# ScissorJack-ever/AlayaLite

Measured on AMD Instinct MI355X. Metric: QPS @ recall@10>=0.95, GIST-960 L2, 1M base / 1k queries, higher is better.
Workload: dtype f32

## Files before the change

### alayalite_amd/csrc/capi.cpp

```cpp
#include "../../include/alaya_hip.h"

#include <hip/hip_runtime_api.h>

#include <algorithm>
#include <cfloat>
#include <cmath>
#include <cstring>
#include <memory>
#include <mutex>
#include <stdexcept>
#include <limits>
#include <string>
#include <thread>
#include <vector>

#include "build_kernels.h"
#include "graph_update.h"
#include "hnsw_build.h"
#include "flat_bound.h"
#include "flat_kernels.h"
#include <cstdlib>
#include "screen_bound.h"
#include "search_kernels.h"

// ... 85 lines not shown
  int sq8_order = 2;
  uint32_t code_stride = 0;
  DevBuf codes, sq_min, sq_max, rr_q_buf, sq_ids, sq_d;
  DevBuf norms, cand_d, cand_i, flat_tau, flag_buf, iota, flat_q;
  DevBuf flat_bias;
  int flat_contraction = -1;
  bool norms_ready = false;
  DevBuf flat_tiles, tiles_cand, tiles_qexp;
  bool tiles_ready = false;
  int tiles_exp = 0;
  int tiles_metric = -1;
  float max_norm = 0.f;
  DevBuf work, overflow, dirty, stab, q_buf, id_buf, dist_buf, cnt_buf, dlist_buf, dout_buf;
  size_t overflow_clean = 0;
  size_t stab_clean = 0;
  uint32_t hash_log2_override = 0;
  int helpers_mode = -1;
  DevBuf help_stats;
  uint64_t help_stats_slots = 0;
  struct ScreenCopy {
    DevBuf rows, err;
    uint64_t cap = 0;
    bool ready = false;
    bool failed = false;
  };
  ScreenCopy screen_copy[2];
  uint32_t screen_format = 0;
  DevBuf screen_stats;
  uint64_t screen_stats_slots = 0;
  uint32_t last_grid = 0, last_waves = 0;
  uint32_t last_lds = 0, last_hash_log2 = 0, last_compact = 0, last_per_cu = 0, last_scout = 0;
  DevBuf scout_stats;
  uint64_t scout_stats_slots = 0;
  int visited_mode_override = 0;
  int num_cus = 0;
  uint64_t capacity = 0;
  std::unique_ptr<alaya_amd::HostGraph> upd_graph;
  std::unique_ptr<alaya_amd::RowMirror> upd_rows;
  std::unique_ptr<alaya_amd::UpdateContext> upd_ctx;
  hipStream_t stream = nullptr;
  hipEvent_t scratch_ev = nullptr;
  hipStream_t scratch_stream = nullptr;
  bool scratch_used = false;
  uint64_t device_bytes() const {
    return base.bytes + valid.bytes + l0.bytes + levels.bytes + upper_off.bytes +
           upper_edges.bytes + eps.bytes + overflow.bytes + dirty.bytes + stab.bytes + codes.bytes + sq_min.bytes +
           sq_max.bytes;
  }
};

namespace {

void set_device(const alaya_index *ix) { hip_check(hipSetDevice(ix->device), "hipSetDevice"); }

void scratch_acquire(alaya_index *ix, hipStream_t s) {
  if (ix->scratch_used && ix->scratch_stream != s)
    hip_check(hipStreamWaitEvent(s, ix->scratch_ev, 0), "hipStreamWaitEvent");
}
void scratch_release(alaya_index *ix, hipStream_t s) {
  hip_check(hipEventRecord(ix->scratch_ev, s), "hipEventRecord");
  ix->scratch_stream = s;
  ix->scratch_used = true;
}
void scratch_suspect(alaya_index *ix) {
  ix->overflow_clean = 0;
  ix->stab_clean = 0;
// ... 209 lines not shown
    } else if (force != 0) {
      int b1 = 0;
      const size_t probe = search_wave_lds_bytes(ix->stride, ef, 12, true);
      hip_check(search_occupancy(resolve_search_variant(r), p.ip, 1, probe, &b1), "occupancy");
      const uint64_t resident1 = static_cast<uint64_t>(std::max(1, b1)) * static_cast<uint64_t>(stream_cus(ix, stream));
      if (nq > resident1 && 2 * nq <= 3 * resident1) r.want |= kModeTwoWaves;
    }
  }
  if (ensure_screen(ix, p, p.sq8_order == 0 && plain, stream)) r.want |= kModeScreen;
  return r;
}

struct SearchPlan {
  const alaya_amd::SearchVariant *variant;
  int W;
  size_t lds;
  int grid;
  int per_cu;
};

uint32_t scout_default(uint32_t dim) { return (dim == 768 || dim == 960) ? alaya_amd::kScoutOn : 0u; }

uint32_t scout_requested(uint32_t dim) {
  const char *e = std::getenv("ALAYA_SEARCH_SCOUT");
  const int asked = e && e[0] ? std::atoi(e) : -1;
  uint32_t f = asked < 0 ? scout_default(dim) : (asked == 1 ? alaya_amd::kScoutOn : (asked == 2 ? alaya_amd::kScoutOn | alaya_amd::kScoutVerify : 0u));
  if (f != 0u) {
    const char *m = std::getenv("ALAYA_SEARCH_SCOUT_MISS");
    if (m && std::atoi(m) != 0) f |= alaya_amd::kScoutMiss;
  }
  return f;
}

SearchPlan plan_search(alaya_index *ix, SearchParams &p, alaya_amd::SearchRequest r, uint64_t nq, uint32_t ef,
                       hipStream_t stream) {
  using namespace alaya_amd;
  SearchPlan plan{};
  for (;;) {
    plan.variant = &resolve_search_variant(r);
    const int mode = plan.variant->mode;
    if ((r.want & kModeStamp) != 0 && (mode & kModeStamp) == 0)
      throw ArgError("no stamped search kernel for dim " + std::to_string(ix->dim) +
                     (p.sq8_order ? " SQ8 (order " + std::to_string(p.sq8_order) + ")" : std::string(" f32")) +
                     ": see the variant list in search_variants.h");
    p.help = (mode & kModeHelp) != 0;
    p.two_waves = (mode & kModeTwoWaves) != 0;
    p.screen = (mode & kModeScreen) != 0 ? ix->screen_format : 0u;
    plan.W = p.help ? 4 : search_waves(p);
    while (!p.help && plan.W > 1 && static_cast<uint64_t>(plan.W) > nq) plan.W /= 2;
    p.hash_log2 = size_visited(ix, p, *plan.variant, nq, ef, plan.W);
    const bool compact = p.vis_rbits != kVisWide;
    p.wave_lds = static_cast<uint32_t>(search_wave_lds_bytes(ix->stride, ef, p.hash_log2, compact, p.sq8_order));
    bool fits = true;
    if (p.help) {
      const size_t need = static_cast<size_t>(plan.W) * kHelpMemoSlots * ix->R * 8;
      const size_t q_bytes = search_query_lds_bytes(ix->stride, p.sq8_order);
      if (q_bytes >= need) {
        p.memo_off = 0;
      } else if (p.wave_lds >= q_bytes + 3 * 64 * 4 + need) {
        p.memo_off = static_cast<uint32_t>(q_bytes + 3 * 64 * 4);
      } else {
        fits = false;
      }
    }
    plan.lds = search_shared_lds_bytes(ix->stride, p.sq8_order != 0) + static_cast<size_t>(plan.W) * p.wave_lds +
               (p.help ? kHelpBoardBytes : 0);
    if (!p.help || (fits && plan.lds <= kLdsPerCu)) break;
    r.want &= ~kModeHelp;
  }
  if (plan.lds > kLdsPerCu) throw ArgError("ef / dim too large for the LDS budget");
  int per_cu = 0;
  hip_check(search_occupancy(*plan.variant, p.ip, plan.W, plan.lds, &per_cu), "occupancy");
  per_cu = static_cast<int>(std::max<uint64_t>(1, std::min<uint64_t>(per_cu, max_search_waves_per_cu() / plan.W)));
  const uint64_t cus = static_cast<uint64_t>(stream_cus(ix, stream));
  const uint64_t blocks_needed = p.help ? static_cast<uint64_t>(per_cu) * cus : (nq + plan.W - 1) / plan.W;
  plan.grid = static_cast<int>(std::max<uint64_t>(1, std::min<uint64_t>(blocks_needed, static_cast<uint64_t>(per_cu) * cus)));
  plan.per_cu = per_cu;
  p.scout = 0u;
  const uint32_t scout = scout_requested(ix->dim);
  if (scout != 0u && p.screen == 3u && !p.ip && !p.two_waves && !p.help && plan.W == 1 && ix->R <= kScoutR &&
      (plan.variant->mode & ~kModeScreen) == 0 && search_has_two_waves(ix->dim, p.sq8_order, ix->generic) &&
      !helpers_requested(ix, p, nq, cus)) {
    SearchRequest r2 = r;
    r2.want |= kModeTwoWaves;
    const SearchVariant &v2 = resolve_search_variant(r2);
    const size_t lds2 = plan.lds + kScoutBoardBytes;
    int per_cu2 = 0;
    if (v2.mode == (kModeScreen | kModeTwoWaves) && lds2 <= kLdsPerCu)
      hip_check(search_occupancy(v2, false, 2, lds2, &per_cu2), "occupancy");
    if (per_cu2 >= per_cu && nq <= static_cast<uint64_t>(per_cu) * cus) {
      plan.variant = &v2;
      plan.lds = lds2;
      p.scout = scout;
      if (const char *e = std::getenv("ALAYA_SEARCH_SCOUT_GRID"))
        plan.grid = std::max(1, std::min(plan.grid, std::atoi(e)));
    }
  }
  return plan;
}

void do_search(alaya_index *ix, const float *d_q, uint64_t nq, uint32_t k, uint32_t ef,
               uint32_t *d_ids, float *d_dists, uint32_t *d_cnt, hipStream_t stream,
               uint64_t *d_stamps = nullptr, bool sq8 = false, uint32_t fill_id = 0) {
  if (!ix->base.ptr) throw ArgError("index has no base vectors");
  if (!ix->has_graph) throw ArgError("index has no graph");
  if (ef == 0) throw ArgError("ef must be >= 1");
  if (k == 0 || nq == 0) return;
  if (ix->graph_n > ix->n) throw ArgError("graph has more nodes than base vectors");
  SearchParams p = base_params(ix);
  p.l0 = ix->l0.as<uint32_t>();
  p.R = ix->R;
  p.dedup_edges = ix->dedup;
  p.levels = ix->has_overlay ? ix->levels.as<uint32_t>() : nullptr;
  p.upper_off = ix->upper_off.as<uint64_t>();
  p.upper_edges = ix->upper_edges.as<uint32_t>();
  p.upper_R = ix->upper_R;
  p.ep = ix->ep;
  p.eps = ix->eps.as<uint32_t>();
  p.n_eps = ix->n_eps;
  p.queries = d_q;
  p.nq = nq;
  p.q_stride = ix->dim;
  p.k = k;
  p.ef = ef;
  p.out_ids = d_ids;
  p.out_dists = d_dists;
// ... 2 lines not shown
  p.fill_id = fill_id;
  if (sq8) {
    if (!ix->has_sq8) throw ArgError("index has no SQ8 codes");
    p.sq8_order = ix->sq8_order;
    p.codes = ix->codes.as<uint8_t>();
    p.code_stride = ix->code_stride;
    p.sq_min = ix->sq_min.as<float>();
    p.sq_max = ix->sq_max.as<float>();
  }
  p.stab_log2 = spill_table_log2(p.sq8_order, std::max<uint32_t>(1, ceil_log2(std::max<uint64_t>(ix->n, 2))), ef);
  if (const char *e = std::getenv("ALAYA_HELP_FLAGS")) p.help_flags = static_cast<uint32_t>(std::strtoul(e, nullptr, 10));
  const SearchPlan plan = plan_search(ix, p, search_request(ix, p, nq, ef, stream), nq, ef, stream);
  if (p.screen >= 2) {
    p.screen_u8 = ix->screen_copy[1].rows.as<uint8_t>();
  } else if (p.screen) {
    p.screen_rows = ix->screen_copy[0].rows.as<uint16_t>();
    p.screen_err = ix->screen_copy[0].err.as<float>();
  }
  scratch_acquire(ix, stream);
  const uint64_t searchers = static_cast<uint64_t>(plan.grid) * plan.W;
  prepare_spill(ix, p, searchers, stream);
  ix->last_grid = static_cast<uint32_t>(plan.grid);
  const int wg_waves = p.scout ? 2 * plan.W : plan.W;
  ix->last_waves = static_cast<uint32_t>(wg_waves);
  ix->last_lds = static_cast<uint32_t>(plan.lds);
  ix->last_hash_log2 = p.hash_log2;
  ix->last_compact = p.vis_rbits != alaya_amd::kVisWide ? 1u : 0u;
  ix->last_per_cu = static_cast<uint32_t>(plan.per_cu);
  ix->last_scout = p.scout;
  ix->scout_stats_slots = p.scout ? searchers : 0;
  if (p.scout) {
    ix->scout_stats.reserve(searchers * 16);
    p.scout_stats = ix->scout_stats.as<uint32_t>();
  }
  ix->help_stats_slots = p.help ? searchers : 0;
  if (p.help) {
    ix->help_stats.reserve(searchers * 12);
    p.help_stats = ix->help_stats.as<uint32_t>();
  }
  ix->screen_stats_slots = p.screen ? searchers : 0;
  if (p.screen) {
    ix->screen_stats.reserve(searchers * 8);
    p.screen_stats = ix->screen_stats.as<uint32_t>();
  }
  ix->work.reserve(4);
  p.work_counter = ix->work.as<uint32_t>();
  hip_check(hipMemsetAsync(p.work_counter, 0, 4, stream), "hipMemsetAsync");
  hip_check(alaya_amd::launch_search(*plan.variant, p, plan.grid, wg_waves, plan.lds, stream), "search launch");
  scratch_release(ix, stream);
}

uint32_t screen_default(uint32_t dim) {
  return (dim == 512 || dim == 768 || dim == 960 || dim == 1024) ? 3u : 0u;
}

void screen_fill(alaya_index *ix, uint32_t format, uint64_t first, uint64_t count, hipStream_t stream) {
  alaya_index::ScreenCopy &c = ix->screen_copy[format - 1];
  hip_check(format == 2 ? alaya_amd::launch_screen_rows_u8(ix->base.as<float>(), first, count, ix->stride,
                                                           c.rows.as<uint8_t>(), stream)
                        : alaya_amd::launch_screen_rows(ix->base.as<float>(), first, count, ix->stride,
                                                        c.rows.as<uint16_t>(), c.err.as<float>(), stream),
            "screening copy");
}

bool ensure_screen(alaya_index *ix, const SearchParams &p, bool eligible, hipStream_t stream) {
  ix->screen_format = 0;
  if (!eligible || !alaya_amd::search_has_screen(ix->dim, p.sq8_order, ix->generic, p.ip)) return false;
// ... 1458 lines not shown
}

int alaya_index_last_plan(const alaya_index *ix, uint32_t *lds_bytes, uint32_t *hash_log2, uint32_t *compact,
                          uint32_t *groups_per_cu, uint32_t *scout) {
  return guarded([&] {
    if (!ix) throw ArgError("null index");
    if (lds_bytes) *lds_bytes = ix->last_lds;
    if (hash_log2) *hash_log2 = ix->last_hash_log2;
    if (compact) *compact = ix->last_compact;
    if (groups_per_cu) *groups_per_cu = ix->last_per_cu;
    if (scout) *scout = ix->last_scout;
  });
}

int alaya_index_scout_stats(alaya_index *ix, uint64_t *expansions, uint64_t *hits, uint64_t *records,
                            uint64_t *mismatches) {
  return guarded_scratch(ix, [&] {
    if (!ix) throw ArgError("null index");
    uint64_t t[4] = {0, 0, 0, 0};
    if (ix->scout_stats_slots) {
      set_device(ix);
      scratch_drain(ix);
      std::vector<uint32_t> h(4 * ix->scout_stats_slots);
      hip_check(hipMemcpy(h.data(), ix->scout_stats.ptr, h.size() * 4, hipMemcpyDeviceToHost), "D2H");
      for (uint64_t i = 0; i < h.size(); ++i) t[i & 3] += h[i];
    }
    if (expansions) *expansions = t[0];
    if (hits) *hits = t[1];
    if (records) *records = t[2];
    if (mismatches) *mismatches = t[3];
  });
}

int alaya_index_set_helpers(alaya_index *ix, int mode) {
  return guarded([&] {
    if (!ix) throw ArgError("null index");
    if (mode < -1 || mode > 1) throw ArgError("helpers mode must be -1 (automatic), 0 (off) or 1 (on)");
    ix->helpers_mode = mode;
  });
}

int alaya_index_help_stats(alaya_index *ix, uint64_t *memo_dists, uint64_t *memo_expansions, uint64_t *helper_rows) {
  return guarded_scratch(ix, [&] {
    if (!ix) throw ArgError("null index");
    uint64_t m = 0, x = 0, r = 0;
    if (ix->help_stats_slots) {
      set_device(ix);
      scratch_drain(ix);
      std::vector<uint32_t> h(3 * ix->help_stats_slots);
      hip_check(hipMemcpy(h.data(), ix->help_stats.ptr, h.size() * 4, hipMemcpyDeviceToHost), "D2H");
      for (uint64_t i = 0; i < ix->help_stats_slots; ++i) {
        m += h[3 * i];
        x += h[3 * i + 1];
        r += h[3 * i + 2];
      }
    }
    if (memo_dists) *memo_dists = m;
    if (memo_expansions) *memo_expansions = x;
    if (helper_rows) *helper_rows = r;
  });
}

int alaya_screen_lower_bound(const float *d_tilde, const float *e_row, uint64_t n, uint32_t dim, float *out) {
  return guarded([&] {
    if (n && (!d_tilde || !e_row || !out)) throw ArgError("invalid arguments");
    for (uint64_t i = 0; i < n; ++i) out[i] = alaya_amd::screen_lower_bound(d_tilde[i], e_row[i], dim);
// ... 156 lines not shown
```

### alayalite_amd/csrc/pybind_module.cpp

```cpp
#include <pybind11/numpy.h>
#include <pybind11/pybind11.h>
#include <pybind11/stl.h>

#include <algorithm>
#include <cmath>
#include <cstring>
#include <fstream>
#include <memory>
#include <queue>
#include <stdexcept>
#include <string>
#include <vector>

#include "../../include/alaya_hip.h"

extern "C" int alaya_index_flat_diag(alaya_index *, const float *, uint64_t, uint32_t, int, uint32_t *, float *,
                                     uint32_t *, uint32_t *, void *);
#include "host_distance.h"

namespace py = pybind11;

namespace alaya_py {

enum class IndexType { FLAT = 0, HNSW = 1, NSG = 2, FUSION = 3, QG = 4 };
// ... 241 lines not shown
    upload();
  }

  uint32_t get_data_dim() const { return dim_; }

  py::array last_counters() const {
    py::array_t<uint32_t> out({static_cast<py::ssize_t>(last_counters_.size() / 4), static_cast<py::ssize_t>(4)});
    std::memcpy(out.mutable_data(), last_counters_.data(), last_counters_.size() * 4);
    return out;
  }
  void set_hash_log2(uint32_t v) { check(alaya_index_set_hash_log2(ix_, v)); }
  void set_visited_mode(int m) { check(alaya_index_set_visited_mode(ix_, m)); }
  void set_helpers(int m) { check(alaya_index_set_helpers(ix_, m)); }
  py::tuple last_launch() {
    uint32_t g = 0, w = 0;
    check(alaya_index_last_launch(ix_, &g, &w));
    return py::make_tuple(g, w);
  }
  py::tuple help_stats() {
    uint64_t m = 0, x = 0, r = 0;
    check(alaya_index_help_stats(ix_, &m, &x, &r));
    return py::make_tuple(m, x, r);
  }
  py::tuple screen_stats() {
    uint64_t a = 0, b = 0;
    check(alaya_index_screen_stats(ix_, &a, &b));
    return py::make_tuple(a, b);
  }
  py::tuple scout_stats() {
    uint64_t e = 0, h = 0, r = 0, m = 0;
    check(alaya_index_scout_stats(ix_, &e, &h, &r, &m));
    return py::make_tuple(e, h, r, m);
  }
  py::dict last_plan() {
    uint32_t g = 0, w = 0, lds = 0, hl = 0, c = 0, pc = 0, sc = 0;
    check(alaya_index_last_launch(ix_, &g, &w));
    check(alaya_index_last_plan(ix_, &lds, &hl, &c, &pc, &sc));
    py::dict d;
    d["workgroups"] = g;
    d["waves_per_group"] = w;
    d["lds_bytes"] = lds;
    d["hash_log2"] = hl;
    d["compact"] = c != 0;
    d["groups_per_cu"] = pc;
    d["scout"] = sc;
    return d;
  }
  void set_rerank_mode(int m) {
    if (m != 1 && m != 2) throw std::invalid_argument("rerank mode must be 1 (reference) or 2 (corrected)");
    rerank_mode_ = m;
  }
  int rerank_mode() const { return rerank_mode_; }
  py::array device_distances(py::array queries, py::array_t<uint32_t> ids) {
    py::array q = prepare_queries(queries);
    py::array_t<uint32_t, py::array::c_style | py::array::forcecast> idc(ids);
    const uint64_t nq = q.shape(0);
    const uint32_t n = static_cast<uint32_t>(idc.size());
    py::array_t<float> out({static_cast<py::ssize_t>(nq), static_cast<py::ssize_t>(n)});
    check(alaya_index_distances(ix_, static_cast<const float *>(q.data()), nq, idc.data(), n,
                                out.mutable_data()));
    return out;
  }
  py::tuple graph_arrays() {
    if (!graph_) throw std::runtime_error("index is not fitted");
    sync_graph();
    uint64_t n, nue;
    uint32_t R, upper_R, ep, max_level, n_eps;
    int has_overlay;
    check(alaya_graph_info(graph_, &n, &R, &has_overlay, &upper_R, &ep, &max_level, &nue, &n_eps));
    py::array_t<uint32_t> l0({static_cast<py::ssize_t>(n), static_cast<py::ssize_t>(R)});
    py::array_t<uint32_t> levels(static_cast<py::ssize_t>(has_overlay ? n : 0));
    py::array_t<uint64_t> off(static_cast<py::ssize_t>(has_overlay ? n : 0));
    py::array_t<uint32_t> ue(static_cast<py::ssize_t>(nue));
    py::array_t<uint32_t> eps(static_cast<py::ssize_t>(n_eps));
    check(alaya_graph_export(graph_, l0.mutable_data(), levels.mutable_data(), off.mutable_data(),
                             ue.mutable_data(), eps.mutable_data()));
    return py::make_tuple(l0, has_overlay ? py::object(levels) : py::none(),
                          has_overlay ? py::object(off) : py::none(), ue, ep, upper_R, eps);
// ... 514 lines not shown
    check(alaya_index_flat_last_contraction(ix_, &c));
    return c;
  }
  void flat_diag(uintptr_t q, uint64_t nq, uint32_t k, int ablate, uintptr_t ids, uintptr_t dists,
                 uintptr_t flags, uintptr_t mc, uintptr_t stream) {
    check(alaya_index_flat_diag(ix_, reinterpret_cast<const float *>(q), nq, k, ablate,
                                reinterpret_cast<uint32_t *>(ids), reinterpret_cast<float *>(dists),
                                reinterpret_cast<uint32_t *>(flags), reinterpret_cast<uint32_t *>(mc),
                                reinterpret_cast<void *>(stream)));
  }
  void set_hash_log2(uint32_t v) { check(alaya_index_set_hash_log2(ix_, v)); }
  void set_visited_mode(int m) { check(alaya_index_set_visited_mode(ix_, m)); }
  void set_helpers(int m) { check(alaya_index_set_helpers(ix_, m)); }
  py::tuple last_launch() {
    uint32_t g = 0, w = 0;
    check(alaya_index_last_launch(ix_, &g, &w));
    return py::make_tuple(g, w);
  }
  py::tuple help_stats() {
    uint64_t m = 0, x = 0, r = 0;
    check(alaya_index_help_stats(ix_, &m, &x, &r));
    return py::make_tuple(m, x, r);
  }
  py::tuple screen_stats() {
    uint64_t a = 0, b = 0;
    check(alaya_index_screen_stats(ix_, &a, &b));
    return py::make_tuple(a, b);
  }
  py::tuple scout_stats() {
    uint64_t e = 0, h = 0, r = 0, m = 0;
    check(alaya_index_scout_stats(ix_, &e, &h, &r, &m));
    return py::make_tuple(e, h, r, m);
  }
  py::dict last_plan() {
    uint32_t g = 0, w = 0, lds = 0, hl = 0, c = 0, pc = 0, sc = 0;
    check(alaya_index_last_launch(ix_, &g, &w));
    check(alaya_index_last_plan(ix_, &lds, &hl, &c, &pc, &sc));
    py::dict d;
    d["workgroups"] = g;
    d["waves_per_group"] = w;
    d["lds_bytes"] = lds;
    d["hash_log2"] = hl;
    d["compact"] = c != 0;
    d["groups_per_cu"] = pc;
    d["scout"] = sc;
    return d;
  }
  py::tuple profile_search(py::array_t<float, py::array::c_style | py::array::forcecast> q, uint32_t k,
                           uint32_t ef, int space) {
    const uint64_t nq = q.shape(0);
    py::array_t<uint32_t> ids({static_cast<py::ssize_t>(nq), static_cast<py::ssize_t>(k)});
    py::array_t<uint32_t> c({static_cast<py::ssize_t>(nq), static_cast<py::ssize_t>(4)});
    py::array_t<uint64_t> st({static_cast<py::ssize_t>(nq), static_cast<py::ssize_t>(8)});
    check(alaya_index_profile_search(ix_, q.data(), nq, k, ef, space, ids.mutable_data(), c.mutable_data(),
                                     st.mutable_data()));
    return py::make_tuple(ids, c, st);
  }
  uint64_t device_bytes() const {
    uint64_t b = 0;
    check(alaya_index_info(ix_, nullptr, nullptr, nullptr, nullptr, &b));
    return b;
  }

 private:
  alaya_index *ix_ = nullptr;
};

}

PYBIND11_MODULE(_alayalitepy, m) {
  using namespace alaya_py;
  m.doc() = "AlayaLite MI355X engine";
  m.attr("__version__") = "0.1.0-mi355x";

  py::enum_<IndexType>(m, "IndexType")
      .value("FLAT", IndexType::FLAT)
      .value("HNSW", IndexType::HNSW)
      .value("NSG", IndexType::NSG)
// ... 32 lines not shown
      .def_readwrite("data_type_", &IndexParams::data_type_)
      .def_readwrite("id_type_", &IndexParams::id_type_)
      .def_readwrite("quantization_type_", &IndexParams::quantization_type_)
      .def_readwrite("metric_", &IndexParams::metric_)
      .def_readwrite("capacity_", &IndexParams::capacity_);

  py::class_<PyIndexInterface, std::shared_ptr<PyIndexInterface>>(m, "PyIndexInterface")
      .def(py::init<IndexParams>(), py::arg("params"))
      .def("to_string", &PyIndexInterface::to_string)
      .def("fit", &PyIndexInterface::fit, py::arg("vectors"), py::arg("ef_construction"), py::arg("num_threads"),
           py::arg("builder") = "host")
      .def("search", &PyIndexInterface::search, py::arg("query"), py::arg("topk"), py::arg("ef"))
      .def("get_data_by_id", &PyIndexInterface::get_data_by_id, py::arg("id"))
      .def("insert", &PyIndexInterface::insert, py::arg("insert_data"), py::arg("ef"))
      .def("remove", &PyIndexInterface::remove, py::arg("id"))
      .def("batch_search", &PyIndexInterface::batch_search, py::arg("queries"), py::arg("topk"),
           py::arg("ef"), py::arg("num_threads"))
      .def("batch_search_with_distance", &PyIndexInterface::batch_search_with_distance,
           py::arg("queries"), py::arg("topk"), py::arg("ef"), py::arg("num_threads"))
      .def("exact_search", &PyIndexInterface::exact_search, py::arg("queries"), py::arg("topk"))
      .def("save", &PyIndexInterface::save, py::arg("index_path"), py::arg("data_path"),
           py::arg("quant_path") = std::string())
      .def("load", &PyIndexInterface::load, py::arg("index_path"), py::arg("data_path"),
           py::arg("quant_path") = std::string())
      .def("get_data_dim", &PyIndexInterface::get_data_dim)
      .def("last_counters", &PyIndexInterface::last_counters)
      .def("set_hash_log2", &PyIndexInterface::set_hash_log2)
      .def("set_visited_mode", &PyIndexInterface::set_visited_mode)
      .def("set_helpers", &PyIndexInterface::set_helpers)
      .def("last_launch", &PyIndexInterface::last_launch)
      .def("help_stats", &PyIndexInterface::help_stats)
      .def("screen_stats", &PyIndexInterface::screen_stats)
      .def("scout_stats", &PyIndexInterface::scout_stats)
      .def("last_plan", &PyIndexInterface::last_plan)
      .def("set_rerank_mode", &PyIndexInterface::set_rerank_mode)
      .def("rerank_mode", &PyIndexInterface::rerank_mode)
      .def("device_distances", &PyIndexInterface::device_distances)
      .def("graph_arrays", &PyIndexInterface::graph_arrays);


  py::class_<Graph, std::shared_ptr<Graph>>(m, "Graph")
      .def_static("build", &Graph::build, py::arg("data"), py::arg("metric") = 0, py::arg("R") = 32u,
                  py::arg("ef_construction") = 100u, py::arg("num_threads") = 1u, py::arg("seed") = 100u)
      .def_static("load", &Graph::load, py::arg("path"), py::arg("id_bytes") = 4)
      .def_static("from_arrays", &Graph::from_arrays, py::arg("l0"), py::arg("levels"), py::arg("upper_off"),
                  py::arg("upper_edges"), py::arg("upper_R"), py::arg("ep"), py::arg("eps") = py::none())
      .def("save", &Graph::save, py::arg("path"), py::arg("id_bytes") = 4, py::arg("capacity") = 0u)
      .def("arrays", &Graph::arrays);
  py::class_<DeviceIndex, std::shared_ptr<DeviceIndex>>(m, "DeviceIndex")
      .def(py::init<int>(), py::arg("device") = 0)
      .def("set_base", &DeviceIndex::set_base, py::arg("rows"), py::arg("metric") = 0, py::arg("valid") = py::none())
      .def("set_graph", &DeviceIndex::set_graph)
      .def("build_graph", &DeviceIndex::build_graph, py::arg("R") = 32, py::arg("ef_construction") = 100,
           py::arg("seed") = 100, py::arg("batch_div") = 0, py::arg("max_batch") = 0, py::arg("refine") = 2)
      .def("search", &DeviceIndex::search, py::arg("queries"), py::arg("k"), py::arg("ef"))
      .def("search_device", &DeviceIndex::search_device)
      .def("shard_search_device", &DeviceIndex::shard_search_device)
      .def("distances", &DeviceIndex::distances)
      .def("set_hash_log2", &DeviceIndex::set_hash_log2)
      .def("set_visited_mode", &DeviceIndex::set_visited_mode)
      .def("set_helpers", &DeviceIndex::set_helpers)
      .def("last_launch", &DeviceIndex::last_launch)
      .def("help_stats", &DeviceIndex::help_stats)
      .def("screen_stats", &DeviceIndex::screen_stats)
      .def("scout_stats", &DeviceIndex::scout_stats)
      .def("last_plan", &DeviceIndex::last_plan)
      .def("flat_search", &DeviceIndex::flat_search, py::arg("queries"), py::arg("k"))
      .def("flat_search_device", &DeviceIndex::flat_search_device)
      .def("flat_diag", &DeviceIndex::flat_diag)
      .def("flat_contraction", &DeviceIndex::flat_contraction)
      .def("search_sq8_device", &DeviceIndex::search_sq8_device)
      .def("shard_search_sq8_device", &DeviceIndex::shard_search_sq8_device)
      .def("set_sq8", &DeviceIndex::set_sq8, py::arg("codes"), py::arg("min"), py::arg("max"), py::arg("order") = 2)
      .def("search_sq8", &DeviceIndex::search_sq8, py::arg("queries"), py::arg("k"), py::arg("ef"),
           py::arg("rerank") = 1, py::arg("rerank_queries") = py::none())
      .def("profile_search", &DeviceIndex::profile_search, py::arg("q"), py::arg("k"), py::arg("ef"),
           py::arg("space") = 0)
      .def("device_bytes", &DeviceIndex::device_bytes);
  m.def("sq8_train", [](py::array_t<float, py::array::c_style | py::array::forcecast> data) {
    const uint32_t d = static_cast<uint32_t>(data.shape(1));
    py::array_t<float> mn(d), mx(d);
    check(alaya_sq8_train(data.data(), data.shape(0), d, mn.mutable_data(), mx.mutable_data()));
    return py::make_tuple(mn, mx);
  });
  m.def("sq8_encode", [](py::array_t<float, py::array::c_style | py::array::forcecast> data,
                         py::array_t<float, py::array::c_style | py::array::forcecast> mn,
                         py::array_t<float, py::array::c_style | py::array::forcecast> mx, uint32_t threads) {
    py::array_t<uint8_t> codes({data.shape(0), data.shape(1)});
    check(alaya_sq8_encode(data.data(), data.shape(0), static_cast<uint32_t>(data.shape(1)), mn.data(), mx.data(),
                           codes.mutable_data(), threads));
    return codes;
  }, py::arg("data"), py::arg("min"), py::arg("max"), py::arg("num_threads") = 1u);
  m.def("host_sq8_order", &host_sq8_order);
  m.def("build_info", [] { return std::string(alaya_build_info()); });
  m.def("screen_lower_bound", [](py::array_t<float, py::array::c_style | py::array::forcecast> d_tilde,
                                 py::array_t<float, py::array::c_style | py::array::forcecast> e_row, uint32_t dim) {
    if (d_tilde.size() != e_row.size()) throw std::invalid_argument("d_tilde and e_row differ in size");
    py::array_t<float> out(d_tilde.size());
// ... 86 lines not shown
```

### alayalite_amd/csrc/search_kernels.h

```cpp
#pragma once
#include <hip/hip_runtime_api.h>

#include <cstddef>
#include <cstdint>

#include "search_variants.h"

namespace alaya_amd {

struct SearchParams {
  const float *base;
  uint64_t n;
  uint32_t dim;
  uint32_t stride;
  const uint32_t *valid;
  bool ip;
  bool generic;
  const uint32_t *l0;
  uint32_t R;
  bool dedup_edges;
  const uint32_t *levels;
  const uint64_t *upper_off;
  const uint32_t *upper_edges;
  uint32_t upper_R;
// ... 11 lines not shown
  uint32_t fill_id;
  uint32_t *work_counter;
  uint32_t *overflow_bits;
  uint32_t *dirty_words;
  uint32_t dirty_cap;
  uint32_t wave_lds;
  uint32_t hash_log2;
  uint32_t vis_rbits;
  uint32_t vis_lbits;
  uint32_t vis_max_disp;
  uint32_t vis_limit;
  uint16_t *spill_table;
  uint32_t stab_log2;
  uint32_t stab_rbits;
  uint32_t spill_flags;
  uint64_t *stamps;
  int sq8_order;
  const uint8_t *codes;
  uint32_t code_stride;
  const float *sq_min;
  const float *sq_max;
  uint32_t help;
  uint32_t help_flags;
  uint32_t memo_off;
  uint32_t two_waves;
  uint32_t *help_stats;
  uint32_t screen;
  const uint16_t *screen_rows;
  const float *screen_err;
  const uint8_t *screen_u8;
  uint32_t *screen_stats;
  uint32_t scout;
  uint32_t *scout_stats;
};
constexpr uint32_t kScoutOn = 1, kScoutVerify = 2, kScoutMiss = 4;
constexpr uint32_t kScoutSlots = 3;
constexpr uint32_t kScoutR = 32;
constexpr size_t kScoutBoardBytes = kScoutSlots * (kScoutR * 4 + 8 + 4) + 20;

struct RerankParams {
  const uint32_t *search_ids;
  uint32_t k;
  uint32_t n_src;
  uint32_t n_take;
  uint32_t zeros;
  uint32_t fill_id;
  uint32_t *out_ids;
  float *out_dists;
};

constexpr uint32_t kVisWide = 0xffffffffu;
constexpr size_t kHelpBoardBytes = 256;
#ifndef ALAYA_HELP_DEPTH
#define ALAYA_HELP_DEPTH 1
#endif
constexpr size_t kHelpMemoSlots = ALAYA_HELP_DEPTH + 1;
constexpr uint32_t kStabBucket = 8;
inline size_t visited_table_bytes(uint32_t hash_log2, bool compact) {
  return (static_cast<size_t>(compact ? 2 : 4)) << hash_log2;
}
size_t search_wave_lds_bytes(uint32_t stride, uint32_t ef, uint32_t hash_log2, bool compact = false,
                             int sq8_order = 0);
size_t search_query_lds_bytes(uint32_t stride, int sq8_order);
__host__ __device__ inline size_t search_shared_lds_bytes(uint32_t stride, bool sq8) {
  return sq8 ? 2 * static_cast<size_t>(stride) * 4 : 0;
}
hipError_t launch_rerank(const SearchParams &p, const RerankParams &r, hipStream_t stream);
hipError_t search_occupancy(const SearchVariant &v, bool ip, int waves, size_t lds, int *blocks_per_cu);
// ... 14 lines not shown
```

### alayalite_amd/csrc/search_kernels.hip

```cpp
#include <hip/hip_runtime.h>

#include <cfloat>
#include <cstdint>

#include "screen_bound.h"
#include "search_kernels.h"
#include "search_device.h"

#ifndef ALAYA_MIN_WAVES_SQ8
#define ALAYA_MIN_WAVES_SQ8 -1
#endif
#ifndef ALAYA_MIN_WAVES_NARROW
#define ALAYA_MIN_WAVES_NARROW 0
#endif
#ifndef ALAYA_MIN_WAVES_WIDE
#define ALAYA_MIN_WAVES_WIDE 0
#endif
template <int kSpace>
constexpr bool space_sq8() { return kSpace == 1 || kSpace == 2; }
template <int kSpace>
constexpr bool space_tab() { return kSpace == 2; }

template <int kChunks, int kSpace, int kMode = 0>
constexpr int search_min_waves() {
// ... 445 lines not shown
  uint32_t bound[kScoutSlots][kScoutR];
  uint32_t req[kScoutSlots];
  uint32_t state;
  uint32_t stat[3];
  uint32_t pad;
};
static_assert(sizeof(ScoutBoard) == kScoutBoardBytes && kScoutSlots == 3, "board size");

__device__ __forceinline__ ScoutBoard *scout_board(const SearchParams &p, unsigned char *smem, int n_search, int i) {
  return reinterpret_cast<ScoutBoard *>(smem + search_shared_lds_bytes(p.stride, p.sq8_order != 0) +
                                        static_cast<size_t>(n_search) * p.wave_lds) + i;
}

template <typename T>
__device__ __forceinline__ T lds_load(const T *a) {
  return __hip_atomic_load(a, __ATOMIC_RELAXED, __HIP_MEMORY_SCOPE_WORKGROUP);
}
template <typename T, typename U>
__device__ __forceinline__ void lds_store(T *a, U v) {
  __hip_atomic_store(a, static_cast<T>(v), __ATOMIC_RELAXED, __HIP_MEMORY_SCOPE_WORKGROUP);
}
__device__ __forceinline__ void lds_order() { asm volatile("" ::: "memory"); }

__device__ __forceinline__ uint64_t scout_key(uint32_t epoch, uint32_t node) {
  return (static_cast<uint64_t>(epoch & 0x7fffffffu) << 32) | node;
}

__device__ __forceinline__ void scout_post(ScoutBoard *b, int first, int n, uint32_t x0, uint32_t x1, uint32_t x2) {
  const int lane = lane_id();
  if (lane < n) lds_store(&b->req[first + lane], lane == 0 ? x0 : (lane == 1 ? x1 : x2));
}

template <int kChunks>
__device__ void scout_loop(const SearchParams &p, const Lds &Ls, ScoutBoard *b, uint32_t *stats) {
  const int lane = lane_id();
  const int mine = screen_pass_row(lane);
  const int R = static_cast<int>(p.R);
  const uint32_t rec = screen_u8_record_bytes(p.stride);
  const bool miss = (p.scout & kScoutMiss) != 0u;
  __builtin_amdgcn_s_setprio(0);
  ScreenQuery sq{};
  uint32_t sq_epoch = 0u;
  uint32_t records = 0u;
  for (;;) {
    const uint32_t e = read_lane(lds_load(&b->state), 0);
    if (e == kScoutDone) break;
    if (e == 0u) {
      __builtin_amdgcn_s_sleep(8);
      continue;
    }
    if (e != sq_epoch) {
      lds_order();
      sq = screen_query_codes<kChunks>(p, Ls.q);
      lds_order();
      sq_epoch = read_lane(lds_load(&b->state), 0) == e ? e : 0u;
      continue;
    }
    uint32_t rq = kEmpty;
    uint64_t tg = 0ull;
    if (lane < static_cast<int>(kScoutSlots)) {
      rq = lds_load(&b->req[lane]);
      tg = lds_load(&b->tag[lane]);
    }
    lds_order();
    if (read_lane(lds_load(&b->state), 0) != sq_epoch) continue;
    const uint32_t u = read_lane(rq, 0), c1 = read_lane(rq, 1), c2 = read_lane(rq, 2);
    const uint64_t ku = scout_key(e, u), k1 = scout_key(e, c1), k2 = scout_key(e, c2);
    tg &= ~kScoutNoMatch;
    const bool have1 = ballot(tg == k1) != 0ull, have2 = ballot(tg == k2) != 0ull;
    uint32_t node = kEmpty;
    if (!miss && c1 != kEmpty && !have1) {
      node = c1;
    } else if (c2 != kEmpty && !have2) {
      node = c2;
    }
    const uint64_t spare = ballot(lane < static_cast<int>(kScoutSlots) && tg != ku && tg != k1 && tg != k2);
    if (node == kEmpty || spare == 0ull) {
      __builtin_amdgcn_s_sleep(8);
      continue;
    }
    const int row = __ffsll(static_cast<unsigned long long>(spare)) - 1;
    const uint32_t v = lane < R ? p.l0[static_cast<uint64_t>(node) * p.R + lane] : kEmpty;
    const uint64_t endm = ballot(lane < R && v == kEmpty);
    const int cnt = endm ? __ffsll(static_cast<unsigned long long>(endm)) - 1 : R;
    bool want = lane < cnt;
    want = want && !sibling_visited<0>(p, Ls, 0, v, want);
    const uint64_t wm = ballot(want);
    if (lane == 0) lds_store(&b->tag[row], 0ull);
    lds_order();
    uint32_t lb_bits = kScoutMissing;
    if (wm != 0ull) {
      const uint32_t v0 = read_lane(v, __ffsll(static_cast<unsigned long long>(wm)) - 1);
      const uint32_t id = want ? v : v0;
      const uint32_t idm = static_cast<uint32_t>(__builtin_amdgcn_ds_bpermute(mine << 2, static_cast<int>(id)));
      const uint8_t *rp = p.screen_u8 + static_cast<uint64_t>(idm) * rec;
      const float4 head = *reinterpret_cast<const float4 *>(rp);
      const uint2 sums = *reinterpret_cast<const uint2 *>(rp + screen_u8_sums_offset(p.stride));
      const uint32_t ac = screen_dots_pass<kChunks>(p, sq.codes, id, NoHook());
      const float lb = screen_int_bound(p.stride, sq.err, sq.lo, sq.scale, sq.a1, sq.a2, head.x, head.y, head.z, sums.x,
                                        sums.y, ac);
      if ((wm >> mine) & 1ull) lb_bits = __float_as_uint(lb);
      records += static_cast<uint32_t>(__popcll(wm));
    }
    if (lane < 32 && mine < R) lds_store(&b->bound[row][mine], lb_bits);
    lds_order();
    if (lane == 0) lds_store(&b->tag[row], scout_key(e, node) | (miss ? kScoutNoMatch : 0ull));
  }
  if (stats != nullptr && lane == 0) stats[2] = records;
}

template <bool kIP, int kChunks, int kMode, int kSpace = 0>
__global__ void __launch_bounds__(256)
    __attribute__((amdgpu_waves_per_eu(search_min_waves<kChunks, kSpace, kMode>() ? search_min_waves<kChunks, kSpace, kMode>() : 1,
                                       8))) hnsw_search_kernel(SearchParams p) {
  extern __shared__ __attribute__((aligned(16))) unsigned char smem[];
  constexpr bool kStamp = (kMode & kModeStamp) != 0;
  constexpr bool kCheck = (kMode & kModeCheck) != 0;
  constexpr bool kHelp = (kMode & kModeHelp) != 0;
  constexpr int kRows = (kMode & kModeTwoWaves) != 0 ? 1 : 0;
  constexpr bool kScreen = (kMode & kModeScreen) != 0;
  static_assert(!kScreen || (kSpace == 0 && !kIP && !kHelp && kChunks >= 16 && kChunks % 2 == 0), "screen: wide f32 L2 rows");
  constexpr int kScreenRows = (kMode & kModeTwoWaves) != 0 ? 2 : 4;
  constexpr int kScreenRowsU8 = 4;
  uint32_t n_screened = 0, n_screened_out = 0;
  const int lane = lane_id();
  const int wave = static_cast<int>(threadIdx.x >> 6);
  constexpr bool kScout = kScreen && (kMode & kModeTwoWaves) != 0;
  const bool scouting = kScout && p.scout != 0u;
  const int W = static_cast<int>(blockDim.x >> 6) >> (scouting ? 1 : 0);
  ScoutBoard *sboard = nullptr;
  if constexpr (kScout) {
    if (scouting) {
      sboard = scout_board(p, smem, W, wave < W ? wave : wave - W);
      if (wave < W && lane < static_cast<int>(kScoutSlots)) {
        sboard->req[lane] = kEmpty;
        sboard->tag[lane] = 0ull;
        sboard->stat[lane] = 0u;
        sboard->state = 0u;
      }
      __syncthreads();
      if (wave >= W) {
        const uint64_t sslot = static_cast<uint64_t>(blockIdx.x) * W + (wave - W);
        scout_loop<kChunks>(p, carve_lds<kSpace>(p, smem, wave - W), sboard,
                            p.scout_stats != nullptr ? p.scout_stats + 4 * sslot : nullptr);
        return;
      }
      __builtin_amdgcn_s_setprio(2);
    }
  }
  const Lds L = carve_lds<kSpace>(p, smem, wave);
  fill_shared<kSpace>(p, L);
  HelpBoard *board = kHelp ? help_board(p, smem, W) : nullptr;
  HelpMine mine;
  if constexpr (kHelp) {
    if constexpr (ALAYA_HELP_PRIO > 0) __builtin_amdgcn_s_setprio(ALAYA_HELP_PRIO);
    if (threadIdx.x == 0) help_board_init(board);
    __syncthreads();
    for (int s = 0; s < kHelpSlots; ++s) mine.node[s] = kEmpty, mine.seq[s] = 0u;
    mine.next_seq = 0u;
    mine.memo_wave = -1;
  }
  const uint64_t bit_words = (p.n + 31) / 32;
  const uint64_t slot = static_cast<uint64_t>(blockIdx.x) * W + wave;
  uint32_t *slot_bits = p.overflow_bits + slot * bit_words;
  uint32_t *slot_dirty = p.dirty_words + slot * p.dirty_cap;
  uint16_t *slot_stab = (space_tab<kSpace>() && p.spill_table) ? p.spill_table + (slot << p.stab_log2) : nullptr;

  bool first_round = true;
  for (;;) {
    uint32_t qi = 0;
    if (kHelp && first_round) {
      qi = static_cast<uint32_t>(wave) * gridDim.x + blockIdx.x;
    } else {
      if (lane == 0) qi = atomicAdd(p.work_counter, 1u);
      qi = read_lane(qi, 0) + (kHelp ? static_cast<uint32_t>(W) * gridDim.x : 0u);
    }
    first_round = false;
// ... 186 lines not shown
              wave_sync();
              screen_dots_int<kChunks>(p, sq.codes, L.cid, nf, reinterpret_cast<uint32_t *>(L.cd), NoHook());
              const float own = screen_int_bound(p.stride, sq.err, sq.lo, sq.scale, sq.a1, sq.a2, head.x, head.y, head.z,
                                                 sums.x, sums.y, __float_as_uint(L.cd[lane]));
              const uint32_t bad = static_cast<uint32_t>(__popcll(ballot(in && __float_as_uint(own) != __float_as_uint(lb3))));
              if (lane == 0 && bad != 0u) sboard->stat[2] += bad;
            }
          } else if (p.screen == 3) {
            if constexpr (kScout) {
              if (scouting && lane == 0) sboard->stat[0] += 1u;
            }
            const uint8_t *rp = p.screen_u8 + static_cast<uint64_t>(c) * screen_u8_record_bytes(p.stride);
            const float4 head = *reinterpret_cast<const float4 *>(rp);
            const uint2 sums = *reinterpret_cast<const uint2 *>(rp + screen_u8_sums_offset(p.stride));
            screen_dots_int<kChunks>(p, sq.codes, L.cid, nf, reinterpret_cast<uint32_t *>(L.cd), second_level_prefetch);
            lb3 = screen_int_bound(p.stride, sq.err, sq.lo, sq.scale, sq.a1, sq.a2, head.x, head.y, head.z, sums.x, sums.y,
                                   __float_as_uint(L.cd[lane]));
          } else if (p.screen == 2) {
            if (in) e_row = *reinterpret_cast<const float *>(p.screen_u8 + static_cast<uint64_t>(c) * screen_u8_record_bytes(p.stride));
            screen_distances_u8<kChunks, kScreenRowsU8>(p, L.q, L.cid, nf, L.cd, second_level_prefetch);
          } else {
            if (in) e_row = p.screen_err[c];
            screen_distances<kChunks, kScreenRows>(p, L.q, L.cid, nf, L.cd, second_level_prefetch);
          }
          bool keep = false;
          if (in) {
            const float lb = p.screen == 3 ? lb3 : screen_lower_bound(L.cd[lane], e_row, p.dim);
            keep = !(lb > 0.f && lb >= tau);
          }
          const uint64_t km = ballot(keep);
          nd = __popcll(km);
          n_screened += static_cast<uint32_t>(nf);
          n_screened_out += static_cast<uint32_t>(nf - nd);
          if (keep) L.cid[__popcll(km & ((1ull << lane) - 1ull))] = c;
          wave_sync();
          if (nd == 0) {
            stamp(3);
            n_dist += nf;
            continue;
          }
        }
      }
      if constexpr (kScreen) {
        constexpr int kFull = RowPass<kChunks, kRows>::kR;
        if (nd <= 8) {
          space_distances<kIP, kChunks, kSpace, false, 1>(p, L, L.cid, nd, L.cd);
        } else if (kFull > 2 && nd <= 16) {
          space_distances<kIP, kChunks, kSpace, false, 2>(p, L, L.cid, nd, L.cd);
        } else {
          space_distances<kIP, kChunks, kSpace, false, kRows>(p, L, L.cid, nd, L.cd);
        }
      } else if (!kHelp || compute) {
        space_distances<kIP, kChunks, kSpace, kHelp, kRows>(p, L, dist_ids, nf, L.cd, second_level_prefetch);
      } else {
        second_level_prefetch();
      }
      stamp(3);
      n_dist += nf;
      const bool has = lane < nd;
      const uint32_t cid = has ? L.cid[lane] : 0u;
      const float cd = has ? L.cd[lane] : 0.f;
      wave_sync();
      pool_merge<kRegMerge>(ps, L, has, cid, cd, [&](uint32_t nx) {
        if (nx != pred) {
          const uint32_t old_pred = pred;
          (void)old_pred;
          pred = nx;
          if (lane < static_cast<int>(p.R)) pred_v = p.l0[static_cast<uint64_t>(nx) * p.R + lane];
          if constexpr (kHelp) {
            if (mine.memo_wave >= 0) mine_request(board, wave, mine, kEmpty, nx, old_pred);
          }
          if constexpr (kScout) {
            if (scouting && ps.size == ps.ef) scout_post(sboard, 1, 2, nx, old_pred, kEmpty);
          }
        }
      }
#ifdef ALAYA_FINE_STAMPS
      , [&]() { stamp(7); }
#endif
      );
      stamp(4);
    }

    query_end(p, L, ps, qi, n_dist, n_expand, n_dist_up, n_hops_up);
    visit_end(vs);
    if constexpr (kStamp) {
      st[6] = __builtin_readcyclecounter() - t_begin;
      if (lane < 8) p.stamps[static_cast<uint64_t>(qi) * 8 + lane] = st[lane & 7];
    }
    wave_sync();
  }
  if constexpr (kHelp) {
    help_siblings<kIP, kChunks, kSpace>(p, smem, L, board, wave, W);
    if (p.help_stats != nullptr && lane == 0) {
      p.help_stats[3 * slot] = board->own[wave].hits;
      p.help_stats[3 * slot + 1] = board->own[wave].skips;
      p.help_stats[3 * slot + 2] = board->own[wave].rows;
    }
  }
  if constexpr (kScout) {
    if (scouting) {
      if (lane == 0) lds_store(&sboard->state, kScoutDone);
      if (p.scout_stats != nullptr && lane == 0) {
        p.scout_stats[4 * slot] = sboard->stat[0];
        p.scout_stats[4 * slot + 1] = sboard->stat[1];
        p.scout_stats[4 * slot + 3] = sboard->stat[2];
      }
    }
  }
  if constexpr (kScreen) {
    if (p.screen_stats != nullptr && lane == 0) {
      p.screen_stats[2 * slot] = n_screened;
      p.screen_stats[2 * slot + 1] = n_screened_out;
    }
  }
}

__global__ void __launch_bounds__(256) screen_rows_kernel(const float *base, uint64_t first, uint64_t count,
                                                          uint32_t stride, uint16_t *out_rows, float *out_err) {
  const int lane = lane_id();
  const uint64_t waves = static_cast<uint64_t>(gridDim.x) * (blockDim.x >> 6);
  for (uint64_t r = static_cast<uint64_t>(blockIdx.x) * (blockDim.x >> 6) + (threadIdx.x >> 6); r < count; r += waves) {
    const float *row = base + (first + r) * stride;
    uint16_t *dst = out_rows + (first + r) * stride;
    float sum = 0.f;
    bool bad = false;
    for (uint32_t e = 2 * lane; e < stride; e += 128) {
      const float2 x = *reinterpret_cast<const float2 *>(row + e);
      const _Float16 h0 = static_cast<_Float16>(x.x), h1 = static_cast<_Float16>(x.y);
      const float y0 = static_cast<float>(h0), y1 = static_cast<float>(h1);
      bad = bad || !(fabsf(y0) <= 65504.f) || !(fabsf(y1) <= 65504.f) || !(fabsf(x.x) <= FLT_MAX) ||
            !(fabsf(x.y) <= FLT_MAX);
      const float d0 = x.x - y0, d1 = x.y - y1;
      sum = fmaf(d0, d0, sum);
      sum = fmaf(d1, d1, sum);
      const half2_t h = {h0, h1};
      *reinterpret_cast<uint32_t *>(dst + e) = __builtin_bit_cast(uint32_t, h);
    }
    sum += lane_xor<1>(sum);
// ... 284 lines not shown
```

### include/alaya_hip.h

```cpp
#ifndef ALAYA_HIP_H_
#define ALAYA_HIP_H_

#include <stddef.h>
#include <stdint.h>

#ifdef __cplusplus
extern "C" {
#endif

#define ALAYA_OK 0
#define ALAYA_ERR_ARG 1
#define ALAYA_ERR_RUNTIME 2
#define ALAYA_ERR_DEVICE 3

#define ALAYA_METRIC_L2 0
#define ALAYA_METRIC_IP 1
#define ALAYA_METRIC_COS 2
#define ALAYA_DIST_GENERIC 0x100

typedef struct alaya_index alaya_index;
typedef struct alaya_graph alaya_graph;

const char *alaya_last_error(void);
const char *alaya_build_info(void);
// ... 62 lines not shown
                                        uint64_t nq, uint32_t k, uint32_t ef, int rerank, uint32_t *d_ids,
                                        float *d_dists, uint32_t *d_counters, void *stream);
int alaya_index_shard_search_sq8_device(alaya_index *ix, const float *d_queries, const float *d_rerank_queries,
                                        uint64_t nq, uint32_t k, uint32_t ef, int holds_row0, uint32_t *d_ids,
                                        float *d_dists, uint32_t *d_counters, void *stream);
int alaya_index_flat_search(alaya_index *ix, const float *queries, uint64_t nq, uint32_t k,
                            uint32_t *ids, float *dists, uint32_t *n_recomputed);
int alaya_index_flat_search_device(alaya_index *ix, const float *d_queries, uint64_t nq, uint32_t k,
                                   uint32_t *d_ids, float *d_dists, uint32_t *d_flags, void *stream);
int alaya_index_flat_last_contraction(const alaya_index *ix, int *contraction);
int alaya_index_set_hash_log2(alaya_index *ix, uint32_t log2_slots);
int alaya_index_set_visited_mode(alaya_index *ix, int mode);
int alaya_index_set_helpers(alaya_index *ix, int mode);
int alaya_index_help_stats(alaya_index *ix, uint64_t *memo_dists, uint64_t *memo_expansions,
                           uint64_t *helper_rows);
int alaya_index_screen_stats(alaya_index *ix, uint64_t *screened, uint64_t *screened_out);
int alaya_screen_lower_bound(const float *d_tilde, const float *e_row, uint64_t n, uint32_t dim, float *out);
int alaya_screen_u8_quantize(const float *rows, uint64_t n, uint32_t dim, uint8_t *codes, float *header,
                             float *values);
int alaya_screen_int_bound(const float *queries, const float *rows, uint64_t n, uint32_t dim, float *d_in,
                           float *e_sum, float *bound, uint32_t *sums);
int alaya_flat_ip_slack(int contraction, uint32_t k_acc, const float *q_norm2, const int *q_exp, uint64_t n,
                        float b_max, int base_exp, float *out);
int alaya_flat_ip_proven(const float *kth_d, const float *cutoff, const float *slack, uint64_t n, uint8_t *out);
int alaya_search_variant(uint32_t dim, int ip, int sq8_order, int generic, uint32_t wanted_mode, int *space,
                         uint32_t *chunks, uint32_t *mode, uint32_t *has_mode);
int alaya_search_variant_at(uint32_t index, int *space, uint32_t *chunks, uint32_t *mode, int *l2_only,
                            uint32_t *count);
int alaya_index_last_launch(const alaya_index *ix, uint32_t *workgroups, uint32_t *waves_per_group);
int alaya_index_last_plan(const alaya_index *ix, uint32_t *lds_bytes, uint32_t *hash_log2, uint32_t *compact,
                          uint32_t *groups_per_cu, uint32_t *scout);
int alaya_index_scout_stats(alaya_index *ix, uint64_t *expansions, uint64_t *hits, uint64_t *records,
                            uint64_t *mismatches);
int alaya_index_info(const alaya_index *ix, uint64_t *n, uint32_t *dim, uint32_t *stride,
                     int *metric, uint64_t *device_bytes);

#ifdef __cplusplus
}
#endif
#endif
```

Baseline: 343,500.

## Post scout prefetch requests early from screening and recheck stale requests

Adds a scout policy, on by default for dims 768 and 960, under which the main search wave posts the best surviving screened candidate to the scout wave as soon as screening finds one that beats the current frontier, rather than only when the next node is chosen. The scout wave also re-reads the board before doing work and drops requests that became stale. The aim is to give the helper wave more lead time to precompute neighbour records, so less of its effort is wasted. The cost is extra cross-lane reductions and LDS traffic on the main wave, possible useless scout work on wrong guesses, and new stats counters kept in the board's pad field.

New measurement: 358,000, median of 6. 1.04x the previous value.

```diff
diff --git a/alayalite_amd/csrc/capi.cpp b/alayalite_amd/csrc/capi.cpp
--- a/alayalite_amd/csrc/capi.cpp
+++ b/alayalite_amd/csrc/capi.cpp
@@ -141,6 +141,8 @@
   uint32_t last_lds = 0, last_hash_log2 = 0, last_compact = 0, last_per_cu = 0, last_scout = 0;
   DevBuf scout_stats;
   uint64_t scout_stats_slots = 0;
+  DevBuf scout_policy_stats;
+  uint32_t last_scout_policy = 0;
   int visited_mode_override = 0;
   int num_cus = 0;
   uint64_t capacity = 0;
@@ -416,6 +418,17 @@
   return f;
 }
 
+uint32_t scout_policy_default(uint32_t dim) {
+  return (dim == 768 || dim == 960) ? (alaya_amd::kScoutEarly | alaya_amd::kScoutRecheck) : 0u;
+}
+
+uint32_t scout_policy_requested(uint32_t dim) {
+  const char *e = std::getenv("ALAYA_SEARCH_SCOUT_POLICY");
+  if (!(e && e[0])) return scout_policy_default(dim);
+  return static_cast<uint32_t>(std::strtoul(e, nullptr, 0)) &
+         (alaya_amd::kScoutEarly | alaya_amd::kScoutRecheck);
+}
+
 SearchPlan plan_search(alaya_index *ix, SearchParams &p, alaya_amd::SearchRequest r, uint64_t nq, uint32_t ef,
                        hipStream_t stream) {
   using namespace alaya_amd;
@@ -461,6 +474,7 @@
   plan.grid = static_cast<int>(std::max<uint64_t>(1, std::min<uint64_t>(blocks_needed, static_cast<uint64_t>(per_cu) * cus)));
   plan.per_cu = per_cu;
   p.scout = 0u;
+  p.scout_policy = 0u;
   const uint32_t scout = scout_requested(ix->dim);
   if (scout != 0u && p.screen == 3u && !p.ip && !p.two_waves && !p.help && plan.W == 1 && ix->R <= kScoutR &&
       (plan.variant->mode & ~kModeScreen) == 0 && search_has_two_waves(ix->dim, p.sq8_order, ix->generic) &&
@@ -476,6 +490,7 @@
       plan.variant = &v2;
       plan.lds = lds2;
       p.scout = scout;
+      p.scout_policy = scout_policy_requested(ix->dim);
       if (const char *e = std::getenv("ALAYA_SEARCH_SCOUT_GRID"))
         plan.grid = std::max(1, std::min(plan.grid, std::atoi(e)));
     }
@@ -544,7 +559,10 @@
   if (p.scout) {
     ix->scout_stats.reserve(searchers * 16);
     p.scout_stats = ix->scout_stats.as<uint32_t>();
-  }
+    ix->scout_policy_stats.reserve(searchers * 12);
+    p.scout_policy_stats = ix->scout_policy_stats.as<uint32_t>();
+  }
+  ix->last_scout_policy = p.scout_policy;
   ix->help_stats_slots = p.help ? searchers : 0;
   if (p.help) {
     ix->help_stats.reserve(searchers * 12);
@@ -2069,6 +2087,25 @@
   });
 }
 
+int alaya_index_scout_policy_stats(alaya_index *ix, uint32_t *policy, uint64_t *early_posts, uint64_t *confirmed,
+                                   uint64_t *abandoned) {
+  return guarded_scratch(ix, [&] {
+    if (!ix) throw ArgError("null index");
+    uint64_t t[3] = {0, 0, 0};
+    if (ix->scout_stats_slots && (early_posts || confirmed || abandoned)) {
+      set_device(ix);
+      scratch_drain(ix);
+      std::vector<uint32_t> h(3 * ix->scout_stats_slots);
+      hip_check(hipMemcpy(h.data(), ix->scout_policy_stats.ptr, h.size() * 4, hipMemcpyDeviceToHost), "D2H");
+      for (uint64_t i = 0; i < h.size(); ++i) t[i % 3] += h[i];
+    }
+    if (policy) *policy = ix->last_scout_policy;
+    if (early_posts) *early_posts = t[0];
+    if (confirmed) *confirmed = t[1];
+    if (abandoned) *abandoned = t[2];
+  });
+}
+
 int alaya_index_set_helpers(alaya_index *ix, int mode) {
   return guarded([&] {
     if (!ix) throw ArgError("null index");
diff --git a/alayalite_amd/csrc/pybind_module.cpp b/alayalite_amd/csrc/pybind_module.cpp
--- a/alayalite_amd/csrc/pybind_module.cpp
+++ b/alayalite_amd/csrc/pybind_module.cpp
@@ -297,6 +297,16 @@
     check(alaya_index_scout_stats(ix_, &e, &h, &r, &m));
     return py::make_tuple(e, h, r, m);
   }
+  py::tuple scout_policy_stats() {
+    uint64_t a = 0, c = 0, d = 0;
+    check(alaya_index_scout_policy_stats(ix_, nullptr, &a, &c, &d));
+    return py::make_tuple(a, c, d);
+  }
+  uint32_t scout_policy() {
+    uint32_t pol = 0;
+    check(alaya_index_scout_policy_stats(ix_, &pol, nullptr, nullptr, nullptr));
+    return pol;
+  }
   py::dict last_plan() {
     uint32_t g = 0, w = 0, lds = 0, hl = 0, c = 0, pc = 0, sc = 0;
     check(alaya_index_last_launch(ix_, &g, &w));
@@ -309,6 +319,7 @@
     d["compact"] = c != 0;
     d["groups_per_cu"] = pc;
     d["scout"] = sc;
+    d["scout_policy"] = scout_policy();
     return d;
   }
   void set_rerank_mode(int m) {
@@ -889,6 +900,16 @@
     check(alaya_index_scout_stats(ix_, &e, &h, &r, &m));
     return py::make_tuple(e, h, r, m);
   }
+  py::tuple scout_policy_stats() {
+    uint64_t a = 0, c = 0, d = 0;
+    check(alaya_index_scout_policy_stats(ix_, nullptr, &a, &c, &d));
+    return py::make_tuple(a, c, d);
+  }
+  uint32_t scout_policy() {
+    uint32_t pol = 0;
+    check(alaya_index_scout_policy_stats(ix_, &pol, nullptr, nullptr, nullptr));
+    return pol;
+  }
   py::dict last_plan() {
     uint32_t g = 0, w = 0, lds = 0, hl = 0, c = 0, pc = 0, sc = 0;
     check(alaya_index_last_launch(ix_, &g, &w));
@@ -901,6 +922,7 @@
     d["compact"] = c != 0;
     d["groups_per_cu"] = pc;
     d["scout"] = sc;
+    d["scout_policy"] = scout_policy();
     return d;
   }
   py::tuple profile_search(py::array_t<float, py::array::c_style | py::array::forcecast> q, uint32_t k,
@@ -999,6 +1021,7 @@
       .def("help_stats", &PyIndexInterface::help_stats)
       .def("screen_stats", &PyIndexInterface::screen_stats)
       .def("scout_stats", &PyIndexInterface::scout_stats)
+      .def("scout_policy_stats", &PyIndexInterface::scout_policy_stats)
       .def("last_plan", &PyIndexInterface::last_plan)
       .def("set_rerank_mode", &PyIndexInterface::set_rerank_mode)
       .def("rerank_mode", &PyIndexInterface::rerank_mode)
@@ -1031,6 +1054,7 @@
       .def("help_stats", &DeviceIndex::help_stats)
       .def("screen_stats", &DeviceIndex::screen_stats)
       .def("scout_stats", &DeviceIndex::scout_stats)
+      .def("scout_policy_stats", &DeviceIndex::scout_policy_stats)
       .def("last_plan", &DeviceIndex::last_plan)
       .def("flat_search", &DeviceIndex::flat_search, py::arg("queries"), py::arg("k"))
       .def("flat_search_device", &DeviceIndex::flat_search_device)
diff --git a/alayalite_amd/csrc/search_kernels.h b/alayalite_amd/csrc/search_kernels.h
--- a/alayalite_amd/csrc/search_kernels.h
+++ b/alayalite_amd/csrc/search_kernels.h
@@ -67,8 +67,11 @@
   uint32_t *screen_stats;
   uint32_t scout;
   uint32_t *scout_stats;
+  uint32_t scout_policy;
+  uint32_t *scout_policy_stats;
 };
 constexpr uint32_t kScoutOn = 1, kScoutVerify = 2, kScoutMiss = 4;
+constexpr uint32_t kScoutEarly = 1, kScoutRecheck = 2;
 constexpr uint32_t kScoutSlots = 3;
 constexpr uint32_t kScoutR = 32;
 constexpr size_t kScoutBoardBytes = kScoutSlots * (kScoutR * 4 + 8 + 4) + 20;
diff --git a/alayalite_amd/csrc/search_kernels.hip b/alayalite_amd/csrc/search_kernels.hip
--- a/alayalite_amd/csrc/search_kernels.hip
+++ b/alayalite_amd/csrc/search_kernels.hip
@@ -501,16 +501,17 @@
 }
 
 template <int kChunks>
-__device__ void scout_loop(const SearchParams &p, const Lds &Ls, ScoutBoard *b, uint32_t *stats) {
+__device__ void scout_loop(const SearchParams &p, const Lds &Ls, ScoutBoard *b, uint32_t *stats, uint32_t *policy_stats) {
   const int lane = lane_id();
   const int mine = screen_pass_row(lane);
   const int R = static_cast<int>(p.R);
   const uint32_t rec = screen_u8_record_bytes(p.stride);
   const bool miss = (p.scout & kScoutMiss) != 0u;
+  const bool recheck = (p.scout_policy & kScoutRecheck) != 0u;
   __builtin_amdgcn_s_setprio(0);
   ScreenQuery sq{};
   uint32_t sq_epoch = 0u;
-  uint32_t records = 0u;
+  uint32_t records = 0u, abandoned = 0u;
   for (;;) {
     const uint32_t e = read_lane(lds_load(&b->state), 0);
     if (e == kScoutDone) break;
@@ -555,6 +556,17 @@
     bool want = lane < cnt;
     want = want && !sibling_visited<0>(p, Ls, 0, v, want);
     const uint64_t wm = ballot(want);
+    if (recheck) {
+      lds_order();
+      uint32_t rq2 = kEmpty;
+      if (lane < static_cast<int>(kScoutSlots)) rq2 = lds_load(&b->req[lane]);
+      lds_order();
+      const uint32_t e2 = read_lane(lds_load(&b->state), 0);
+      if (e2 != e || (read_lane(rq2, 1) != node && read_lane(rq2, 2) != node)) {
+        ++abandoned;
+        continue;
+      }
+    }
     if (lane == 0) lds_store(&b->tag[row], 0ull);
     lds_order();
     uint32_t lb_bits = kScoutMissing;
@@ -576,6 +588,7 @@
     if (lane == 0) lds_store(&b->tag[row], scout_key(e, node) | (miss ? kScoutNoMatch : 0ull));
   }
   if (stats != nullptr && lane == 0) stats[2] = records;
+  if (policy_stats != nullptr && lane == 0) policy_stats[2] = abandoned;
 }
 
 template <bool kIP, int kChunks, int kMode, int kSpace = 0>
@@ -596,6 +609,7 @@
   const int wave = static_cast<int>(threadIdx.x >> 6);
   constexpr bool kScout = kScreen && (kMode & kModeTwoWaves) != 0;
   const bool scouting = kScout && p.scout != 0u;
+  const bool early = scouting && p.screen == 3 && (p.scout_policy & kScoutEarly) != 0u;
   const int W = static_cast<int>(blockDim.x >> 6) >> (scouting ? 1 : 0);
   ScoutBoard *sboard = nullptr;
   if constexpr (kScout) {
@@ -606,12 +620,14 @@
         sboard->tag[lane] = 0ull;
         sboard->stat[lane] = 0u;
         sboard->state = 0u;
+        sboard->pad = 0u;
       }
       __syncthreads();
       if (wave >= W) {
         const uint64_t sslot = static_cast<uint64_t>(blockIdx.x) * W + (wave - W);
         scout_loop<kChunks>(p, carve_lds<kSpace>(p, smem, wave - W), sboard,
-                            p.scout_stats != nullptr ? p.scout_stats + 4 * sslot : nullptr);
+                            p.scout_stats != nullptr ? p.scout_stats + 4 * sslot : nullptr,
+                            p.scout_policy_stats != nullptr ? p.scout_policy_stats + 3 * sslot : nullptr);
         return;
       }
       __builtin_amdgcn_s_setprio(2);
@@ -864,6 +880,22 @@
           nd = __popcll(km);
           n_screened += static_cast<uint32_t>(nf);
           n_screened_out += static_cast<uint32_t>(nf - nd);
+          if constexpr (kScout) {
+            if (early && nd > 0 && ps.cur < ps.size) {
+              const uint32_t kb = keep ? (lb3 > 0.f ? __float_as_uint(lb3) : 0u) : 0xffffffffu;
+              uint32_t mn = min(kb, lane_xor<1>(kb));
+              mn = min(mn, lane_xor<2>(mn));
+              mn = min(mn, lane_xor<4>(mn));
+              mn = min(mn, lane_xor<8>(mn));
+              mn = min(mn, lane_xor<16>(mn));
+              mn = min(read_lane(mn, 0), read_lane(mn, 32));
+              if (__uint_as_float(mn) < L.pd[ps.cur]) {
+                const uint32_t cand = read_lane(c, __ffsll(static_cast<unsigned long long>(ballot(kb == mn))) - 1);
+                scout_post(sboard, 1, 2, cand, pred, kEmpty);
+                if (lane == 0 && (sboard->pad & 0xffffu) != 0xffffu) sboard->pad += 1u;
+              }
+            }
+          }
           if (keep) L.cid[__popcll(km & ((1ull << lane) - 1ull))] = c;
           wave_sync();
           if (nd == 0) {
@@ -903,7 +935,12 @@
             if (mine.memo_wave >= 0) mine_request(board, wave, mine, kEmpty, nx, old_pred);
           }
           if constexpr (kScout) {
-            if (scouting && ps.size == ps.ef) scout_post(sboard, 1, 2, nx, old_pred, kEmpty);
+            if (scouting && ps.size == ps.ef) {
+              if (early && lane == 0 && lds_load(&sboard->req[1]) == nx &&
+                  (sboard->pad >> 16) != 0xffffu)
+                sboard->pad += 0x10000u;
+              scout_post(sboard, 1, 2, nx, old_pred, kEmpty);
+            }
           }
         }
       }
@@ -937,6 +974,10 @@
         p.scout_stats[4 * slot] = sboard->stat[0];
         p.scout_stats[4 * slot + 1] = sboard->stat[1];
         p.scout_stats[4 * slot + 3] = sboard->stat[2];
+      }
+      if (p.scout_policy_stats != nullptr && lane == 0) {
+        p.scout_policy_stats[3 * slot] = sboard->pad & 0xffffu;
+        p.scout_policy_stats[3 * slot + 1] = sboard->pad >> 16;
       }
     }
   }
diff --git a/include/alaya_hip.h b/include/alaya_hip.h
--- a/include/alaya_hip.h
+++ b/include/alaya_hip.h
@@ -118,6 +118,8 @@
                           uint32_t *groups_per_cu, uint32_t *scout);
 int alaya_index_scout_stats(alaya_index *ix, uint64_t *expansions, uint64_t *hits, uint64_t *records,
                             uint64_t *mismatches);
+int alaya_index_scout_policy_stats(alaya_index *ix, uint32_t *policy, uint64_t *early_posts, uint64_t *confirmed,
+                                   uint64_t *abandoned);
 int alaya_index_info(const alaya_index *ix, uint64_t *n, uint32_t *dim, uint32_t *stride,
                      int *metric, uint64_t *device_bytes);
 
```
